# greysun/GraphEmbeddings

Hardware: AMD Instinct MI355X
Metric: scored triples/sec/GPU (d=200) (higher is better)
Workload: dtype f32

## Files before the change

graphembeddings_amd/csrc/ge_train.hip:

```cpp
#include "ge_prep.h"
#include "ge_launch.h"
#include <algorithm>
#include <cmath>
#include <utility>

namespace ge {

__global__ __launch_bounds__(kPrepThreads) void train_prepare_kernel(
    const int32_t* __restrict__ triples, int64_t T, int64_t first_row, int64_t B, int64_t s0,
    const int32_t* __restrict__ id_to_type, int64_t N, const int64_t* __restrict__ type_offsets,
    int32_t n_types, const int32_t* __restrict__ type_ids, uint64_t seed, uint64_t global_step0,
    int32_t padded_size, int32_t mode, int direct, int n_pass, int bits, int negs, int32_t* __restrict__ prep) {
  extern __shared__ __attribute__((aligned(16))) unsigned long long keys[];
  const PrepLayout L = prep_layout(B, negs);
  const int P = (int)L.P, R = P / kPrepThreads;
  unsigned* hist = reinterpret_cast<unsigned*>(keys + P);
  int* wtot = reinterpret_cast<int*>(hist + kPrepWaves * kMaxRadix);
  const int tid = threadIdx.x, lane = tid & (kWave - 1), wave = tid >> 6;
  const int sub = blockIdx.y;
  const int64_t s = s0 + blockIdx.x;
  const int32_t* pos = triples + 3 * step_row(first_row, T, B, s);
  int32_t* rec = prep + (int64_t)blockIdx.x * L.stride;
  int32_t* neg = rec;
  int32_t* slot_item = rec + L.off_slot;
  int32_t* subrec = rec + L.off_sub + sub * L.sub_stride;
  int32_t* items = subrec + L.off_items;
  int32_t* islots = subrec + L.off_islots;
  const int64_t i0 = (int64_t)sub * kSub;
  const int S = (int)((L.units - i0) < kSub ? (L.units - i0) : kSub);
  const uint64_t step = global_step0 + (uint64_t)s;
  const bool batch_heads = (mode == GE_CORRUPT_BATCH_COIN) ? batch_coin_heads(seed, step) : false;
  constexpr unsigned long long kInvalid = ~0ull;

  if (direct)
    for (int i = tid; i < 6 * S; i += kPrepThreads) slot_item[6 * i0 + i] = -1;

  {
    const StepSource src{pos, B, id_to_type, N, type_offsets, n_types, type_ids, seed, step, padded_size, mode, negs};
    for (int il = tid; il < (int)L.S; il += kPrepThreads) {
      unsigned long long k4[4] = {kInvalid, kInvalid, kInvalid, kInvalid};
      if (il < S) unit_keys(src, i0 + il, batch_heads, neg, k4);
      if (negs > 0) {
#pragma unroll
        for (int X = 0; X < 3; ++X) keys[3 * il + X] = k4[X];
      } else {
#pragma unroll
        for (int X = 0; X < 4; ++X) keys[4 * il + X] = k4[X];
      }
    }
  }
  __syncthreads();

  const int radix = 1 << bits;
  const unsigned dmask = (unsigned)radix - 1u;
  const int seg = kWave * R;
  for (int pass = 0; pass < n_pass; ++pass) {
    const int shift = 32 + pass * bits;
    for (int i = tid; i < radix * kPrepWaves; i += kPrepThreads) hist[i] = 0;
    __syncthreads();
    unsigned long long k[16];
    unsigned off[16];
#pragma unroll
    for (int r = 0; r < 16; ++r) {
      if (r < R) {
        k[r] = keys[wave * seg + r * kWave + lane];
        const unsigned dg = (unsigned)(k[r] >> shift) & dmask;
        unsigned long long peers = ~0ull;
        for (int b = 0; b < bits; ++b) {
          const bool bit = (dg >> b) & 1u;
          const unsigned long long bal = __ballot(bit);
          peers &= bit ? bal : ~bal;
        }
        const unsigned rank = (unsigned)__popcll(peers & ((1ull << lane) - 1ull));
        const unsigned cnt = (unsigned)__popcll(peers);
        unsigned* hp = hist + dg * kPrepWaves + wave;
        const unsigned base = *hp;
        __builtin_amdgcn_wave_barrier();
        if (rank == 0) *hp = base + cnt;
        __builtin_amdgcn_wave_barrier();
        off[r] = base + rank;
      }
    }
    __syncthreads();
    {
      const int q = radix * kPrepWaves / kPrepThreads;
      unsigned loc[4];
      int sum = 0;
      for (int u = 0; u < q; ++u) { loc[u] = hist[tid * q + u]; sum += (int)loc[u]; }
      const int incl = wave_incl_add(sum, lane);
      if (lane == kWave - 1) wtot[wave] = incl;
      __syncthreads();
      int run = incl - sum;
      for (int w = 0; w < wave; ++w) run += wtot[w];
      for (int u = 0; u < q; ++u) { hist[tid * q + u] = (unsigned)run; run += (int)loc[u]; }
    }
    __syncthreads();
#pragma unroll
    for (int r = 0; r < 16; ++r) {
      if (r < R) {
        const unsigned dg = (unsigned)(k[r] >> shift) & dmask;
        keys[hist[dg * kPrepWaves + wave] + off[r]] = k[r];
      }
    }
    __syncthreads();
  }

  auto key_at = [&](int i) -> unsigned long long { return (i >= 0 && i < P) ? keys[i] : kInvalid; };
  int rs_loc[16];
  {
    int carry = -1;
#pragma unroll
    for (int r = 0; r < 16; ++r) {
      if (r < R) {
        const int i = wave * seg + r * kWave + lane;
        const unsigned long long kk = keys[i], kp = key_at(i - 1);
        const bool head = kk != kInvalid && (i == 0 || (uint32_t)(kp >> 32) != (uint32_t)(kk >> 32));
        const int m = max(wave_incl_max(head ? i : -1, lane), carry);
        rs_loc[r] = m;
        carry = __shfl(m, kWave - 1, kWave);
      }
    }
    if (lane == 0) wtot[wave] = carry;
  }
  __syncthreads();
  int prev_max = -1;
  for (int w = 0; w < wave; ++w) prev_max = max(prev_max, wtot[w]);
  __syncthreads();
  unsigned start_mask = 0;
  int idx_loc[16];
  {
    int carry = 0;
#pragma unroll
    for (int r = 0; r < 16; ++r) {
      if (r < R) {
        const int i = wave * seg + r * kWave + lane;
        const unsigned long long kk = keys[i], kp = key_at(i - 1), kn = key_at(i + 1);
        const bool valid = kk != kInvalid;
        const uint32_t row = (uint32_t)(kk >> 32);
        const bool head = valid && (i == 0 || (uint32_t)(kp >> 32) != row);
        const bool sole = direct && head && !(kn != kInvalid && (uint32_t)(kn >> 32) == row);
        const int rs = max(rs_loc[r], prev_max);
        rs_loc[r] = rs;
        const bool start = valid && ((i - rs) % kItemCap) == 0 && !sole;
        if (start) start_mask |= 1u << r;
        if (sole) slot_item[(uint32_t)kk] = kSlotDirect;
        const int incl = wave_incl_add(start ? 1 : 0, lane) + carry;
        idx_loc[r] = incl - (start ? 1 : 0);
        carry = __shfl(incl, kWave - 1, kWave);
      }
    }
    if (lane == 0) wtot[wave] = carry;
  }
  __syncthreads();
  int prev_items = 0, total = 0;
  for (int w = 0; w < kPrepWaves; ++w) { if (w < wave) prev_items += wtot[w]; total += wtot[w]; }
  if (tid == 0) subrec[0] = total;
#pragma unroll
  for (int r = 0; r < 16; ++r) {
    if (r < R && ((start_mask >> r) & 1u)) {
      const int i = wave * seg + r * kWave + lane;
      const uint32_t row = (uint32_t)(keys[i] >> 32);
      const int idx = prev_items + idx_loc[r];
      int e = i + 1;
      while (e < P && (e - i) < kItemCap && keys[e] != kInvalid && (uint32_t)(keys[e] >> 32) == row) ++e;
      const bool more = (e < P && keys[e] != kInvalid && (uint32_t)(keys[e] >> 32) == row);
      const bool multi = (i != rs_loc[r]) || more;
      items[2 * idx] = (int32_t)row;
      items[2 * idx + 1] = (e - i) | (multi ? (1 << 30) : 0);
#pragma unroll
      for (int j = 0; j < kItemCap; ++j)
        islots[idx * kItemCap + j] = (i + j < e) ? (int32_t)(uint32_t)keys[i + j] : -1;
    }
  }
}

template <int NJ, bool COND, bool DET = false>
__global__ __launch_bounds__(kBlock) void apply_sorted_kernel(
    float* __restrict__ table, int d, const int32_t* __restrict__ sub0, int64_t sub_stride, int off_items,
    int off_islots, const int32_t* __restrict__ grad_idx, const float* grad_val, int split,
    float* __restrict__ out2) {
  const int lane = threadIdx.x & (kWave - 1);
  const int wave = (int)(((int64_t)blockIdx.x * blockDim.x + threadIdx.x) >> 6);
  const int nwaves = (int)(((int64_t)gridDim.x * blockDim.x) >> 6);
  const int32_t* subrec = sub0 + (int64_t)blockIdx.y * sub_stride;
  const int32_t* items = subrec + off_items;
  const int32_t* islots = subrec + off_islots;
  const int n_items = subrec[0];
  for (int w = wave; w < n_items; w += nwaves) {
    const int row = items[2 * w], cm = items[2 * w + 1];
    int slot_v = (lane < kItemCap) ? islots[w * kItemCap + lane] : -1;
    const int cnt = cm & 0x3FFFFFFF;
    const bool multi = (cm >> 30) & 1;
    const bool away = row >= split;
    float* dst = away ? out2 + (int64_t)(row - split) * d : table + (int64_t)row * d;
    float base[NJ];
#pragma unroll
    for (int j = 0; j < NJ; ++j) {
      const int c = lane + kWave * j;
      base[j] = (!multi && !away && c < d) ? dst[c] : 0.f;
    }
    const bool act_v = slot_v >= 0 && (!grad_idx || grad_idx[slot_v] >= 0);
    if (slot_v < 0) slot_v = 0;
    const unsigned long long live = __ballot(act_v);
    const bool park = DET && multi && !away;
    if (live == 0ull && !(away && !multi) && !park) continue;
    float acc[NJ];
#pragma unroll
    for (int j = 0; j < NJ; ++j) acc[j] = 0.f;
    for (int o = 0; o < cnt; o += 4) {
      int sl[4];
      bool on[4];
#pragma unroll
      for (int q = 0; q < 4; ++q) {
        const int src_lane = (o + q < cnt) ? (o + q) : o;
        sl[q] = __shfl(slot_v, src_lane, kWave);
        on[q] = (o + q < cnt) && ((live >> (o + q)) & 1ull);
      }
      float v[4][NJ];
#pragma unroll
      for (int q = 0; q < 4; ++q) {
        const float* src = grad_val + (int64_t)sl[q] * d;
#pragma unroll
        for (int j = 0; j < NJ; ++j) {
          const int c = lane + kWave * j;
          v[q][j] = (c < d && (!COND || on[q])) ? src[c] : 0.f;
        }
      }
#pragma unroll
      for (int q = 0; q < 4; ++q)
#pragma unroll
        for (int j = 0; j < NJ; ++j) acc[j] += on[q] ? v[q][j] : 0.f;
    }
    float* parked = const_cast<float*>(grad_val) + (int64_t)__shfl(slot_v, 0, kWave) * d;
#pragma unroll
    for (int j = 0; j < NJ; ++j) {
      const int c = lane + kWave * j;
      if (c < d) {
        if (park) parked[c] = acc[j];
        else if (multi) atomic_add_f32(dst + c, acc[j]);
        else dst[c] = base[j] + acc[j];
      }
    }
  }
}

constexpr int kHotBlock = 512;
template <int NJ>
__global__ __launch_bounds__(kHotBlock) void hot_rows_kernel(
    float* __restrict__ table, int d, const int32_t* __restrict__ sub0, int64_t sub_stride, int off_items, int off_islots,
    int n_sub, const float* __restrict__ grad_val) {
  constexpr int kScan = kWave;
  constexpr int kWv = kHotBlock / kWave;
  __shared__ int heads[kScan];
  __shared__ int n_heads;
  __shared__ float part[kWv - 1][NJ * kWave];
  const int t = threadIdx.x, lane = t & (kWave - 1), wv = t >> 6, tile = blockIdx.y;
  auto sub_of = [&](int tl) { return sub0 + (int64_t)tl * sub_stride; };
  const int32_t* subrec = sub_of(tile);
  const int n_items = subrec[0];
  for (int win = blockIdx.x; win * kScan < n_items; win += gridDim.x) {
  if (t == 0) n_heads = 0;
  __syncthreads();
  const int k = win * kScan + t;
  if (t < kScan && k < n_items) {
    const int32_t* items = subrec + off_items;
    const int row = items[2 * k], cm = items[2 * k + 1];
    if ((cm >> 30) & 1) {
      int prev_row = -1;
      if (k > 0) prev_row = items[2 * (k - 1)];
      else if (tile > 0) { const int32_t* ps = sub_of(tile - 1); const int pn = ps[0]; if (pn > 0) prev_row = ps[off_items + 2 * (pn - 1)]; }
      if (prev_row != row) heads[atomicAdd(&n_heads, 1)] = k;
    }
  }
  __syncthreads();
  const int nh = n_heads;
  auto item_at = [&](int k0, int r, int row, int& first_slot) -> bool {
    int idx = k0 + r, tl = tile;
    const int32_t* sr = subrec;
    int ni = n_items;
    while (idx >= ni) {
      idx -= ni; ++tl;
      if (tl >= n_sub) return false;
      sr = sub_of(tl); ni = sr[0];
    }
    first_slot = sr[off_islots + idx * kItemCap];
    return sr[off_items + 2 * idx] == row;
  };
  constexpr int kInFlight = NJ <= 4 ? 16 : 8;
  auto add_rows = [&](int fs, int n, float (&acc)[NJ]) {
    for (int o = 0; o < n; o += kInFlight) {
      float v[kInFlight][NJ];
#pragma unroll
      for (int q = 0; q < kInFlight; ++q)
        if (o + q < n) {
          const float* src = grad_val + (int64_t)__shfl(fs, o + q, kWave) * d;
#pragma unroll
          for (int j = 0; j < NJ; ++j) { const int c = lane + kWave * j; v[q][j] = src[c < d ? c : 0]; }
        }
#pragma unroll
      for (int q = 0; q < kInFlight; ++q)
        if (o + q < n) {
#pragma unroll
          for (int j = 0; j < NJ; ++j) acc[j] += v[q][j];
        }
    }
  };
  for (int h = wv; h < nh; h += kWv) {
    const int k0 = heads[h];
    const int row = (subrec + off_items)[2 * k0];
    int fs = 0;
    const bool mine = item_at(k0, lane, row, fs);
    const int n = __popcll(__ballot(mine));
    if (n == kWave) continue;
    float acc[NJ];
#pragma unroll
    for (int j = 0; j < NJ; ++j) acc[j] = 0.f;
    add_rows(fs, n, acc);
    float* dst = table + (int64_t)row * d;
#pragma unroll
    for (int j = 0; j < NJ; ++j) { const int c = lane + kWave * j; if (c < d) dst[c] = dst[c] + acc[j]; }
    if (lane == 0) heads[h] = -1;
  }
  __syncthreads();
  for (int h = 0; h < nh; ++h) {
    const int k0 = heads[h];
    if (k0 < 0) continue;
    const int row = (subrec + off_items)[2 * k0];
// ... 183 lines not shown
      for (int q = 0; q < RG; ++q)
        if (o + q < cnt && ((live >> (o + q)) & 1ull)) {
          const int sl = __builtin_amdgcn_readlane(slot_v, o + q);
          const float* src = grad_val + (int64_t)sl * d;
#pragma unroll
          for (int j = 0; j < NJ; ++j) load_vec<VW>(src + col[j], v[q][j]);
        }
#pragma unroll
      for (int q = 0; q < RG; ++q)
        if (o + q < cnt && ((live >> (o + q)) & 1ull)) {
#pragma unroll
          for (int j = 0; j < NJ; ++j)
#pragma unroll
            for (int e = 0; e < VW; ++e) acc[j][e] += v[q][j][e];
        }
    }
    if (live == 0ull && !away) continue;
#pragma unroll
    for (int j = 0; j < NJ; ++j) {
      if (!ok[j]) continue;
      float o_[VW];
#pragma unroll
      for (int e = 0; e < VW; ++e) o_[e] = base[j][e] + acc[j][e];
      store_vec<VW>(dst + col[j], o_);
    }
  }
}

int apply_items_launch(float* table, int d, const TileGeom& G, const int32_t* step_rec, const int32_t* gidx,
                       const float* gval, int split, float* out2, hipStream_t st, hipEvent_t ev_start, hipEvent_t ev_stop,
                       int det) {
  const int grid = grid_for(G.P, kBlock / kWave);
  const int nj = (d + kWave - 1) / kWave;
  const dim3 g((unsigned)grid, (unsigned)G.n_sub);
  auto hot = [&]() -> int {
    const dim3 gh((unsigned)((G.P + kWave - 1) / kWave), (unsigned)G.n_sub);
#define LH(NJ) hipLaunchKernelGGL((hot_rows_kernel<NJ>), gh, dim3(kHotBlock), 0, st, table, d, step_rec + G.off_sub, G.sub_stride, G.off_items, G.off_islots, G.n_sub, gval)
    if (nj <= 1) LH(1); else if (nj <= 2) LH(2); else if (nj <= 4) LH(4); else if (nj <= 8) LH(8); else LH(16);
#undef LH
    return launch_status();
  };
  if (det && nj > 16) return GE_ENOTSUP;
#define LA(NJ)                                                                                                             \
  {                                                                                                                        \
    if (G.n_sub > 1) hipExtLaunchKernelGGL((apply_sorted_kernel<NJ, true>), g, dim3(kBlock), 0, st, ev_start, ev_stop, 0, table, d, step_rec + G.off_sub, G.sub_stride, G.off_items, G.off_islots, gidx, gval, split, out2); \
    else if (det) { hipExtLaunchKernelGGL((apply_sorted_kernel<NJ, false, true>), g, dim3(kBlock), 0, st, ev_start, ev_stop, 0, table, d, step_rec + G.off_sub, G.sub_stride, G.off_items, G.off_islots, gidx, gval, split, out2); return hot(); } \
    else hipExtLaunchKernelGGL((apply_sorted_kernel<NJ, false>), g, dim3(kBlock), 0, st, ev_start, ev_stop, 0, table, d, step_rec + G.off_sub, G.sub_stride, G.off_items, G.off_islots, gidx, gval, split, out2); \
  }
  if (gidx != nullptr || G.n_sub > 1) {
    auto al = [](const void* q, int a) { return q == nullptr || reinterpret_cast<uintptr_t>(q) % a == 0; };
    const int vw = (d % 4 == 0 && al(table, 16) && al(gval, 16) && al(out2, 16)) ? 4 : (d % 2 == 0 && al(table, 8) && al(gval, 8) && al(out2, 8)) ? 2 : 1;
    const int njr = (d / vw + kWave - 1) / kWave;
    const dim3 g((unsigned)(G.n_sub > 1 ? grid_for((G.P + 7) / 8, kBlock / kWave) : grid), (unsigned)G.n_sub);
    const bool one_tile = G.n_sub == 1 && out2 == nullptr;
#define LR(VW, NJ)                                                                                                       \
    {                                                                                                                    \
      if (one_tile) {                                                                                                    \
        constexpr int RW = one_tile_rows(VW * NJ);                                                                       \
        if (det) {                                                                                                       \
          hipExtLaunchKernelGGL((apply_rows_kernel<VW, NJ, true, RW>), g, dim3(kBlock), 0, st, ev_start, ev_stop, 0, table, d, \
                                step_rec + G.off_sub, G.sub_stride, G.off_items, G.off_islots, gidx, gval, split, out2); \
          return hot();                                                                                                  \
        }                                                                                                                \
        hipExtLaunchKernelGGL((apply_rows_kernel<VW, NJ, false, RW>), g, dim3(kBlock), 0, st, ev_start, ev_stop, 0, table, d, \
                              step_rec + G.off_sub, G.sub_stride, G.off_items, G.off_islots, gidx, gval, split, out2);   \
        return launch_status();                                                                                          \
      }                                                                                                                  \
      if (det) {                                                                                                         \
        hipExtLaunchKernelGGL((apply_rows_kernel<VW, NJ, true>), g, dim3(kBlock), 0, st, ev_start, ev_stop, 0, table, d, \
                              step_rec + G.off_sub, G.sub_stride, G.off_items, G.off_islots, gidx, gval, split, out2);   \
        return hot();                                                                                                    \
      }                                                                                                                  \
      hipExtLaunchKernelGGL((apply_rows_kernel<VW, NJ>), g, dim3(kBlock), 0, st, ev_start, ev_stop, 0, table, d, \
                            step_rec + G.off_sub, G.sub_stride, G.off_items, G.off_islots, gidx, gval, split, out2);     \
      return launch_status();                                                                                            \
    }
    if (vw == 4) { if (njr <= 1) LR(4, 1) else if (njr <= 2) LR(4, 2) else if (njr <= 4) LR(4, 4) }
    else if (vw == 2) { if (njr <= 1) LR(2, 1) else if (njr <= 2) LR(2, 2) else if (njr <= 4) LR(2, 4) else if (njr <= 8) LR(2, 8) }
    else { if (njr <= 1) LR(1, 1) else if (njr <= 2) LR(1, 2) else if (njr <= 4) LR(1, 4) else if (njr <= 8) LR(1, 8) else if (njr <= 16) LR(1, 16) }
#undef LR
  }
  if (nj <= 1) LA(1) else if (nj <= 2) LA(2) else if (nj <= 4) LA(4) else if (nj <= 8) LA(8) else if (nj <= 16) LA(16)
  else return GE_ENOTSUP;
#undef LA
  return launch_status();
}

static int apply_sorted_launch(float* table, int d, const PrepLayout& L, const int32_t* step_rec, const int32_t* gidx,
                               const float* gval, hipStream_t st, hipEvent_t ev_start, hipEvent_t ev_stop, int det = 0) {
  return apply_items_launch(table, d, geom_of(L), step_rec, gidx, gval, 0x7FFFFFFF, nullptr, st, ev_start, ev_stop, det);
}

static size_t grad_region_bytes(int64_t B, int32_t d) {
  return align_up(sizeof(float) * 6 * (size_t)B * (size_t)d, 256);
}
HingeWs hinge_ws(void* base, int64_t B, int32_t d) {
  const size_t idx = align_up(sizeof(int32_t) * 6 * (size_t)B, 256);
  return HingeWs{ws_at<int32_t>(base, 0), ws_at<float>(base, idx), idx + grad_region_bytes(B, d)};
}

static bool train_fast_ok(int64_t B, int32_t d) { return B >= 1 && B <= (int64_t)1 << 24 && d <= 1024; }

static int64_t prep_chunk_steps(int64_t B, int64_t negs = 0) {
  const int64_t u = negs > 0 ? (1 + negs) * B : B;
  int64_t c = (32 * kSub) / (u < kSub ? kSub : u);
  const int64_t floor_steps = u <= 32768 ? 16 : u <= 4 * 65536 ? 8 : 2;
  return c < floor_steps ? floor_steps : c;
}

static int grad_ring(int64_t B, int32_t d) {
  const size_t reg = grad_region_bytes(B, d);
  size_t r = ((size_t)64 << 20) / reg + 1;
  if (r < 2) r = 2;
  if (r > 16) r = 16;
  if (r < 4 && 4 * reg <= ((size_t)160 << 20)) r = 4;
  return (int)r;
}
static size_t prep_chunk_bytes(int64_t B, int64_t negs = 0) {
  return align_up(sizeof(int32_t) * (size_t)prep_chunk_steps(B, negs) * (size_t)prep_layout(B, negs).stride, 256);
}
static size_t prep_region_bytes(int64_t B, int64_t negs) {
  return 2 * prep_chunk_bytes(B, negs) + prep_big_scratch_bytes(B, negs, prep_chunk_steps(B, negs));
}
struct TrainWs { HingeWs g; int ring; size_t region_floats; int32_t* prep; size_t bytes; };
static TrainWs train_ws(void* base, int64_t B, int32_t d) {
  const HingeWs g = hinge_ws(base, B, d);
  const size_t region = grad_region_bytes(B, d);
  const int ring = grad_ring(B, d);
  const size_t grad = g.bytes + (size_t)(ring - 1) * region;
  return TrainWs{g, ring, region / sizeof(float), ws_at<int32_t>(base, grad), grad + prep_region_bytes(B, 0)};
}
template <class Need, class Step>
static size_t largest_need_up_to(int64_t B, Need need, Step step) {
  size_t best = need(B);
  int64_t b = 1;
  while (b < B) {
    const auto v = step(b);
    if (step(B) == v) break;
    int64_t lo = b, hi = B;
    while (hi - lo > 1) { const int64_t mid = lo + (hi - lo) / 2; if (step(mid) == v) lo = mid; else hi = mid; }
    best = std::max(best, need(lo));
    b = hi;
  }
  return best;
}

size_t train_ws_bytes(int64_t B, int32_t d) {
  if (!train_fast_ok(B, d)) return hinge_ws(nullptr, B, d).bytes;
  return largest_need_up_to(B, [&](int64_t b) { return train_ws(nullptr, b, d).bytes; },
                            [&](int64_t b) { return std::make_pair(prep_chunk_steps(b), (int64_t)grad_ring(b, d)); });
}

static size_t prep_lds_bytes(const PrepLayout& L) {
  return sizeof(unsigned long long) * (size_t)L.P + sizeof(unsigned) * kPrepWaves * kMaxRadix + sizeof(int) * 32;
}

static int prepare_launch(const StepSeq& q, int64_t s0, int64_t n, const TypeSampler& ts, int direct, int32_t* out,
                          void* scratch, hipStream_t st, int negs = 0) {
  const PrepLayout L = prep_layout(q.B, negs);
  if (L.n_sub > 1)
    return prepare_big_launch(q, s0, n, ts, direct, out, scratch, st, negs);
  const SortBits sb = sort_bits_for(ts.N);
  const int n_pass = sb.n_pass, bits = sb.bits;
  const size_t lds = prep_lds_bytes(L);
  hipError_t e = hipFuncSetAttribute(reinterpret_cast<const void*>(train_prepare_kernel),
                                     hipFuncAttributeMaxDynamicSharedMemorySize, 160 * 1024);
  if (e != hipSuccess) return (int)e;
  hipLaunchKernelGGL(train_prepare_kernel, dim3((unsigned)n, (unsigned)L.n_sub), dim3(kPrepThreads), lds, st, q.triples,
                     q.T, q.first_row, q.B, s0, ts.id_to_type, ts.N, ts.type_offsets, ts.n_types, ts.type_ids, ts.seed,
                     q.global_step0, ts.padded_size, ts.mode, direct, n_pass, bits, negs, out);
  return launch_status();
}

#define GE_HIP_TRY(expr) do { hipError_t e_ = (expr); if (e_ != hipSuccess) return (int)e_; } while (0)

struct Pipeline {
  int device = -1;
  hipStream_t side = nullptr;
  hipEvent_t prep_done[2] = {nullptr, nullptr};
  hipEvent_t buf_free[2] = {nullptr, nullptr};
  bool live = false;
  StepIdentity id = {};
  int64_t next_abs = 0, resident[2] = {-1, -1};
};

int pipeline_create(void** out) {
  Pipeline* p = new Pipeline();
  hipError_t e = hipGetDevice(&p->device);
  if (e == hipSuccess) e = hipStreamCreateWithFlags(&p->side, hipStreamNonBlocking);
  for (int i = 0; i < 2 && e == hipSuccess; ++i) {
    e = hipEventCreateWithFlags(&p->prep_done[i], hipEventDisableTiming);
    if (e == hipSuccess) e = hipEventCreateWithFlags(&p->buf_free[i], hipEventDisableTiming);
  }
  if (e != hipSuccess) { delete p; return (int)e; }
  *out = p;
  return 0;
}
int pipeline_reset(void* h) {
  if (!h) return GE_EINVAL;
  static_cast<Pipeline*>(h)->live = false;
  return 0;
}
int pipeline_destroy(void* h) {
  if (!h) return GE_EINVAL;
  Pipeline* p = static_cast<Pipeline*>(h);
  if (p->side) { (void)hipStreamSynchronize(p->side); (void)hipStreamDestroy(p->side); }
  for (int i = 0; i < 2; ++i) {
    if (p->prep_done[i]) (void)hipEventDestroy(p->prep_done[i]);
    if (p->buf_free[i]) (void)hipEventDestroy(p->buf_free[i]);
  }
  delete p;
  return 0;
}

static inline int64_t norm_row(int64_t first_row, int64_t T, int64_t B) {
  int64_t f = first_row % T;
  if (f + B > T) f = 0;
  return f;
}
static inline bool continues(const StepSeq& a, int64_t done, const StepSeq& b) {
  return b.global_step0 == a.global_step0 + (uint64_t)done &&
         norm_row(b.first_row, b.T, b.B) == step_row(a.first_row, b.T, b.B, done);
}

class PrepCursor {
 public:
  PrepCursor(const StepIdentity& id, Pipeline* handle, int32_t* prep_base, hipStream_t st)
      : id_(id), L_(prep_layout(id.seq.B, id.negs)), K_(prep_chunk_steps(id.seq.B, id.negs)),
        buf_ints_((int64_t)(prep_chunk_bytes(id.seq.B, id.negs) / sizeof(int32_t))), base_(prep_base), st_(st),
        pipe_(handle ? handle : &local_), own_side_(handle != nullptr) {
    id_.seq.first_row = norm_row(id.seq.first_row, id.seq.T, id.seq.B);
  }

  int begin() {
    if (own_side_) {
      int dev = -1;
      GE_HIP_TRY(hipGetDevice(&dev));
      if (dev != pipe_->device) return GE_EINVAL;
      Pipeline* p = pipe_;
      const bool cont = p->live && same_source(p->id, id_) && continues(p->id.seq, p->next_abs, id_.seq);
      if (!cont) {
        p->live = true;
        p->id = id_;
        p->next_abs = 0;
        p->resident[0] = p->resident[1] = -1;
      }
      base_abs_ = p->next_abs;
    } else {
      pipe_->id = id_;
      pipe_->side = st_;
    }
    return 0;
  }

  int step(int64_t s, const int32_t** rec) {
    const int64_t abs_s = base_abs_ + s, chunk = abs_s / K_, in_chunk = abs_s % K_;
    if (s == 0 || in_chunk == 0) {
      int rc = ensure(chunk);
      if (rc) return rc;
      if (own_side_) {
        rc = ensure(chunk + 1);
        if (rc) return rc;
        GE_HIP_TRY(hipStreamWaitEvent(st_, pipe_->prep_done[chunk & 1], 0));
      }
    }
    *rec = base_ + (chunk & 1) * buf_ints_ + in_chunk * L_.stride;
    return 0;
  }

  int finish(int64_t n_steps, const int32_t** last_rec) {
    const int64_t la = base_abs_ + n_steps - 1;
    *last_rec = base_ + ((la / K_) & 1) * buf_ints_ + (la % K_) * L_.stride;
    if (own_side_) {
      GE_HIP_TRY(hipStreamWaitEvent(st_, pipe_->prep_done[((la / K_) + 1) & 1], 0));
      pipe_->next_abs = base_abs_ + n_steps;
    }
    return 0;
  }

  const PrepLayout& layout() const { return L_; }

 private:
  int ensure(int64_t c) {
    const int b = (int)(c & 1);
    if (pipe_->resident[b] == c) return 0;
    if (own_side_) {
      GE_HIP_TRY(hipEventRecord(pipe_->buf_free[b], st_));
      GE_HIP_TRY(hipStreamWaitEvent(pipe_->side, pipe_->buf_free[b], 0));
    }
    int rc = prepare_launch(pipe_->id.seq, c * K_, K_, id_.ts, id_.direct, base_ + b * buf_ints_, base_ + 2 * buf_ints_,
                            pipe_->side, id_.negs);
    if (rc) return rc;
    if (own_side_) GE_HIP_TRY(hipEventRecord(pipe_->prep_done[b], pipe_->side));
    pipe_->resident[b] = c;
    return 0;
  }

  StepIdentity id_;
  PrepLayout L_;
  int64_t K_, buf_ints_;
  int32_t* base_;
  hipStream_t st_;
  Pipeline local_;
  Pipeline* pipe_;
  bool own_side_;
  int64_t base_abs_ = 0;
};

int train_steps_run(float* table, int32_t d, const StepSeq& q, int64_t n_steps, const TypeSampler& ts, float margin,
                    const StepHyper& hp, int model, float* loss, int keep_all_losses, int32_t* neg_ws, void* workspace,
                    size_t workspace_bytes, void** ev_pairs, int ev_kernel, void* pipe_handle, hipStream_t st) {
  const int64_t N = ts.N, B = q.B;
  const float max_norm = hp.max_norm;
  if (n_steps <= 0) return 0;
  const int deterministic = (model & GE_STEP_DETERMINISTIC) ? 1 : 0;
  model &= ~GE_STEP_DETERMINISTIC;
  const bool shape_ok = complex_shape_ok(d, table);
  const bool transform = model == GE_MODEL_HOLE && shape_ok;
  const bool spectral = transform || model == GE_MODEL_HOLE_SPECTRAL;
  const bool hole_direct = (model == GE_MODEL_HOLE && !shape_ok) || model == GE_MODEL_HOLE_DIRECT;
  if (hole_direct ? d > hole_max_dim() : !shape_ok) return (!hole_direct && (d & 1)) ? GE_EINVAL : GE_ENOTSUP;
  if (transform) { int rc = hole_spectral_launch(table, N, d, 0, st); if (rc) return rc; }
  struct BackToReal {
// ... 206 lines not shown
```

Measured before the change: 597.9 million.

## Restructure prep kernel: narrow 32-bit sort keys, padded LDS, batched sampling, scatter islots

Templates the prepare kernel on key width and radix bits. When the row and slot bit widths fit, it packs sort keys into 32 bits, which halves LDS traffic in the radix sort. It pads LDS and histogram indexing to cut bank conflicts. Negative sampling is batched across several units per thread so the dependent global loads can overlap. Run detection moves to contiguous per-thread segments, and islots are written through a scatter instead of a per-item while loop. The risks are added complexity and correctness of the new item indexing.

```diff
diff --git a/graphembeddings_amd/csrc/ge_train.hip b/graphembeddings_amd/csrc/ge_train.hip
--- a/graphembeddings_amd/csrc/ge_train.hip
+++ b/graphembeddings_amd/csrc/ge_train.hip
@@ -6,17 +6,112 @@
 
 namespace ge {
 
+#ifdef GE_EXP_PREP_STAMPS
+constexpr int kPrepStampWords = 16;
+__device__ unsigned long long ge_prep_stamps[64 * kPrepStampWords];
+#define PREP_STAMP(n) do { if (threadIdx.x == 0 && blockIdx.x < 64) ge_prep_stamps[blockIdx.x * kPrepStampWords + (n)] = __builtin_amdgcn_s_memtime(); } while (0)
+#define PREP_WALL(n) do { if (threadIdx.x == 0 && blockIdx.x < 64) ge_prep_stamps[blockIdx.x * kPrepStampWords + (n)] = wall_clock64(); } while (0)
+#define PREP_STAMP_SYNC() __syncthreads()
+#else
+#define PREP_STAMP(n) do { } while (0)
+#define PREP_WALL(n) do { } while (0)
+#define PREP_STAMP_SYNC() do { } while (0)
+#endif
+
+constexpr int kPrepUnits = (int)(kSub / kPrepThreads);
+constexpr uint32_t kNoSlot = ~0u;
+__host__ __device__ constexpr int prep_pad(int i) { return i + (i >> 4); }
+static_assert(kPrepWaves == 16, "histogram rows are addressed as 17 dg + wave");
+
+template <int BITS>
+__device__ __forceinline__ unsigned long long digit_peers(unsigned dg) {
+  uint32_t diff_lo = 0, diff_hi = 0;
+#pragma unroll
+  for (int b = 0; b < BITS; ++b) {
+    const uint32_t mine = (uint32_t)__builtin_amdgcn_sbfe((int)dg, b, 1);
+    const unsigned long long bal = __ballot(mine != 0u);
+    diff_lo |= (uint32_t)bal ^ mine;
+    diff_hi |= (uint32_t)(bal >> 32) ^ mine;
+  }
+  return ~(((unsigned long long)diff_hi << 32) | diff_lo);
+}
+
+__device__ __forceinline__ void draw_units(const StepSource& S, const int64_t (&j)[kPrepUnits], const bool (&on)[kPrepUnits],
+                                           bool batch_heads, int32_t (&p)[kPrepUnits][3], int (&col)[kPrepUnits],
+                                           int32_t (&repl)[kPrepUnits], bool (&drawn)[kPrepUnits], int64_t (&pi)[kPrepUnits],
+                                           int64_t (&kk)[kPrepUnits]) {
+  const uint32_t klo = (uint32_t)S.seed, khi = (uint32_t)(S.seed >> 32);
+  uint64_t stepk[kPrepUnits];
+#pragma unroll
+  for (int u = 0; u < kPrepUnits; ++u) {
+    pi[u] = (S.negs > 0 && j[u] >= S.B) ? (j[u] - S.B) % S.B : j[u];
+    kk[u] = (S.negs > 0 && j[u] >= S.B) ? (j[u] - S.B) / S.B : 0;
+    drawn[u] = on[u] && (S.negs == 0 || j[u] >= S.B);
+    stepk[u] = S.negs > 0 ? S.step * (uint64_t)S.negs + (uint64_t)kk[u] : S.step;
+#pragma unroll
+    for (int X = 0; X < 3; ++X) p[u][X] = on[u] ? S.pos[3 * pi[u] + X] : -1;
+  }
+  int32_t ty[kPrepUnits];
+  bool ok[kPrepUnits];
+#pragma unroll
+  for (int u = 0; u < kPrepUnits; ++u) {
+    const uint32_t slo = (uint32_t)stepk[u], shi = (uint32_t)(stepk[u] >> 32);
+    const uint32_t ilo = (uint32_t)pi[u], ihi = (uint32_t)((uint64_t)pi[u] >> 32);
+    bool heads;
+    if (S.mode == GE_CORRUPT_BATCH_COIN) heads = S.negs > 0 ? batch_coin_heads(S.seed, stepk[u]) : batch_heads;
+    else if (S.mode == GE_CORRUPT_ROW_COIN) heads = (philox_w0(slo, shi, ilo, ihi, klo ^ GE_TAG_SIDE, khi) >> 31) == 0;
+    else heads = (S.mode == GE_CORRUPT_HEADS);
+    col[u] = heads ? 0 : 1;
+    const int32_t x = heads ? p[u][0] : p[u][1];
+    ok[u] = drawn[u] && x >= 0 && x < S.N;
+    ty[u] = ok[u] ? S.id_to_type[x] : -1;
+  }
+  int64_t off[kPrepUnits], end[kPrepUnits];
+#pragma unroll
+  for (int u = 0; u < kPrepUnits; ++u) {
+    ok[u] = ok[u] && ty[u] >= 0 && ty[u] < S.n_types;
+    off[u] = ok[u] ? S.type_offsets[ty[u]] : 0;
+    end[u] = ok[u] ? S.type_offsets[ty[u] + 1] : 0;
+  }
+  int64_t pick[kPrepUnits];
+#pragma unroll
+  for (int u = 0; u < kPrepUnits; ++u) {
+    const uint32_t slo = (uint32_t)stepk[u], shi = (uint32_t)(stepk[u] >> 32);
+    const uint32_t ilo = (uint32_t)pi[u], ihi = (uint32_t)((uint64_t)pi[u] >> 32);
+    uint32_t w = philox_w0(slo, shi, ilo, ihi, klo ^ GE_TAG_SLOT, khi);
+    if (S.padded_size > 0) {
+      const uint32_t slot = w % (uint32_t)S.padded_size;
+      w = philox_w0(slo, shi, (uint32_t)ty[u], slot, klo ^ GE_TAG_PICK, khi);
+    }
+    const uint64_t len = (uint64_t)(end[u] - off[u]);
+    ok[u] = ok[u] && len > 0;
+    pick[u] = off[u] + (int64_t)(((uint64_t)w * len) >> 32);
+  }
+#pragma unroll
+  for (int u = 0; u < kPrepUnits; ++u)
+    repl[u] = ok[u] ? S.type_ids[pick[u]] : -1;
+}
+
+template <class KeyT, int BITS>
 __global__ __launch_bounds__(kPrepThreads) void train_prepare_kernel(
     const int32_t* __restrict__ triples, int64_t T, int64_t first_row, int64_t B, int64_t s0,
     const int32_t* __restrict__ id_to_type, int64_t N, const int64_t* __restrict__ type_offsets,
     int32_t n_types, const int32_t* __restrict__ type_ids, uint64_t seed, uint64_t global_step0,
-    int32_t padded_size, int32_t mode, int direct, int n_pass, int bits, int negs, int32_t* __restrict__ prep) {
-  extern __shared__ __attribute__((aligned(16))) unsigned long long keys[];
+    int32_t padded_size, int32_t mode, int direct, int n_pass, int sbits, int negs, int32_t* __restrict__ prep) {
+  extern __shared__ __attribute__((aligned(16))) unsigned char prep_lds[];
+  constexpr int bits = BITS;
+  KeyT* keys = reinterpret_cast<KeyT*>(prep_lds);
+  uint32_t* words = reinterpret_cast<uint32_t*>(prep_lds);
   const PrepLayout L = prep_layout(B, negs);
   const int P = (int)L.P, R = P / kPrepThreads;
-  unsigned* hist = reinterpret_cast<unsigned*>(keys + P);
-  int* wtot = reinterpret_cast<int*>(hist + kPrepWaves * kMaxRadix);
+  const int PW = prep_pad(P);
+  unsigned* hist = reinterpret_cast<unsigned*>(prep_lds + sizeof(unsigned long long) * (size_t)PW);
+  int* wtot = reinterpret_cast<int*>(hist + (kPrepWaves + 1) * kMaxRadix);
   const int tid = threadIdx.x, lane = tid & (kWave - 1), wave = tid >> 6;
+  const int rshift = sizeof(KeyT) == 8 ? 32 : sbits;
+  const uint32_t smask = sizeof(KeyT) == 8 ? ~0u : ((1u << sbits) - 1u);
+  PREP_WALL(0);
+  PREP_STAMP(1);
   const int sub = blockIdx.y;
   const int64_t s = s0 + blockIdx.x;
   const int32_t* pos = triples + 3 * step_row(first_row, T, B, s);
@@ -30,16 +125,58 @@
   const int S = (int)((L.units - i0) < kSub ? (L.units - i0) : kSub);
   const uint64_t step = global_step0 + (uint64_t)s;
   const bool batch_heads = (mode == GE_CORRUPT_BATCH_COIN) ? batch_coin_heads(seed, step) : false;
-  constexpr unsigned long long kInvalid = ~0ull;
-
-  if (direct)
-    for (int i = tid; i < 6 * S; i += kPrepThreads) slot_item[6 * i0 + i] = -1;
+  constexpr KeyT kInvalid = (KeyT)~(KeyT)0;
+
+  if (direct) {
+    int32_t* f = slot_item + 6 * i0;
+    const int n = 6 * S;
+    const int head = min(n, (int)((16u - ((uint32_t)reinterpret_cast<uintptr_t>(f) & 15u)) & 15u) >> 2);
+    const int nv = (n - head) >> 2;
+    int4* f4 = reinterpret_cast<int4*>(f + head);
+    for (int i = tid; i < nv; i += kPrepThreads) f4[i] = make_int4(-1, -1, -1, -1);
+    if (tid < head) f[tid] = -1;
+    if (tid < n - head - 4 * nv) f[head + 4 * nv + tid] = -1;
+  }
 
   {
     const StepSource src{pos, B, id_to_type, N, type_offsets, n_types, type_ids, seed, step, padded_size, mode, negs};
-    for (int il = tid; il < (int)L.S; il += kPrepThreads) {
-      unsigned long long k4[4] = {kInvalid, kInvalid, kInvalid, kInvalid};
-      if (il < S) unit_keys(src, i0 + il, batch_heads, neg, k4);
+    int64_t j[kPrepUnits], pi[kPrepUnits], kk[kPrepUnits];
+    bool on[kPrepUnits], drawn[kPrepUnits];
+    int32_t p[kPrepUnits][3], repl[kPrepUnits];
+    int col[kPrepUnits];
+#pragma unroll
+    for (int u = 0; u < kPrepUnits; ++u) {
+      const int il = tid + u * kPrepThreads;
+      on[u] = il < S;
+      j[u] = i0 + (on[u] ? il : 0);
+    }
+    draw_units(src, j, on, batch_heads, p, col, repl, drawn, pi, kk);
+#pragma unroll
+    for (int u = 0; u < kPrepUnits; ++u) {
+      const int il = tid + u * kPrepThreads;
+      if (il >= (int)L.S) continue;
+      KeyT k4[4] = {kInvalid, kInvalid, kInvalid, kInvalid};
+      if (on[u]) {
+        const int32_t old = col[u] ? p[u][1] : p[u][0];
+        int32_t t3[3] = {p[u][0], p[u][1], p[u][2]};
+        if (drawn[u]) {
+          if (col[u]) t3[1] = repl[u]; else t3[0] = repl[u];
+          int32_t* o = neg + 3 * (negs > 0 ? kk[u] * B + pi[u] : j[u]);
+          o[0] = t3[0]; o[1] = t3[1]; o[2] = t3[2];
+        }
+        bool bad = t3[0] < 0 || t3[1] < 0 || t3[2] < 0 || t3[0] >= N || t3[1] >= N || t3[2] >= N;
+        if (negs > 0) {
+#pragma unroll
+          for (int X = 0; X < 3; ++X)
+            if (!bad) k4[X] = ((KeyT)(uint32_t)t3[X] << rshift) | (KeyT)(uint32_t)(3 * j[u] + X);
+        } else {
+          bad = bad || old < 0 || old >= N;
+#pragma unroll
+          for (int X = 0; X < 3; ++X)
+            if (!bad) k4[X] = ((KeyT)(uint32_t)p[u][X] << rshift) | (KeyT)(uint32_t)(6 * j[u] + X);
+          if (!bad && repl[u] != old) k4[3] = ((KeyT)(uint32_t)repl[u] << rshift) | (KeyT)(uint32_t)(6 * j[u] + 3 + col[u]);
+        }
+      }
       if (negs > 0) {
 #pragma unroll
         for (int X = 0; X < 3; ++X) keys[3 * il + X] = k4[X];
@@ -50,30 +187,27 @@
     }
   }
   __syncthreads();
+  PREP_STAMP(2);
 
   const int radix = 1 << bits;
   const unsigned dmask = (unsigned)radix - 1u;
   const int seg = kWave * R;
   for (int pass = 0; pass < n_pass; ++pass) {
-    const int shift = 32 + pass * bits;
-    for (int i = tid; i < radix * kPrepWaves; i += kPrepThreads) hist[i] = 0;
+    const int shift = rshift + pass * bits;
+    const bool last_pass = pass == n_pass - 1;
+    for (int i = tid; i < radix * (kPrepWaves + 1); i += kPrepThreads) hist[i] = 0;
     __syncthreads();
-    unsigned long long k[16];
+    KeyT k[16];
     unsigned off[16];
 #pragma unroll
     for (int r = 0; r < 16; ++r) {
       if (r < R) {
         k[r] = keys[wave * seg + r * kWave + lane];
         const unsigned dg = (unsigned)(k[r] >> shift) & dmask;
-        unsigned long long peers = ~0ull;
-        for (int b = 0; b < bits; ++b) {
-          const bool bit = (dg >> b) & 1u;
-          const unsigned long long bal = __ballot(bit);
-          peers &= bit ? bal : ~bal;
-        }
+        const unsigned long long peers = digit_peers<BITS>(dg);
         const unsigned rank = (unsigned)__popcll(peers & ((1ull << lane) - 1ull));
         const unsigned cnt = (unsigned)__popcll(peers);
-        unsigned* hp = hist + dg * kPrepWaves + wave;
+        unsigned* hp = hist + ((dg << 4) + dg) + wave;
         const unsigned base = *hp;
         __builtin_amdgcn_wave_barrier();
         if (rank == 0) *hp = base + cnt;
@@ -82,97 +216,129 @@
       }
     }
     __syncthreads();
+    if (pass == 0) PREP_STAMP(7);
     {
       const int q = radix * kPrepWaves / kPrepThreads;
       unsigned loc[4];
       int sum = 0;
-      for (int u = 0; u < q; ++u) { loc[u] = hist[tid * q + u]; sum += (int)loc[u]; }
+      for (int u = 0; u < q; ++u) { loc[u] = hist[prep_pad(tid * q + u)]; sum += (int)loc[u]; }
       const int incl = wave_incl_add(sum, lane);
       if (lane == kWave - 1) wtot[wave] = incl;
       __syncthreads();
       int run = incl - sum;
       for (int w = 0; w < wave; ++w) run += wtot[w];
-      for (int u = 0; u < q; ++u) { hist[tid * q + u] = (unsigned)run; run += (int)loc[u]; }
+      for (int u = 0; u < q; ++u) { hist[prep_pad(tid * q + u)] = (unsigned)run; run += (int)loc[u]; }
     }
     __syncthreads();
+    if (pass == 0) PREP_STAMP(8);
 #pragma unroll
     for (int r = 0; r < 16; ++r) {
       if (r < R) {
         const unsigned dg = (unsigned)(k[r] >> shift) & dmask;
-        keys[hist[dg * kPrepWaves + wave] + off[r]] = k[r];
+        const int dst = (int)(hist[((dg << 4) + dg) + wave] + off[r]);
+        keys[last_pass ? prep_pad(dst) : dst] = k[r];
       }
     }
     __syncthreads();
-  }
-
-  auto key_at = [&](int i) -> unsigned long long { return (i >= 0 && i < P) ? keys[i] : kInvalid; };
-  int rs_loc[16];
+    if (pass == 0) PREP_STAMP(9);
+  }
+
+  PREP_STAMP(3);
+  const int p0 = tid * R;
+  KeyT k[16];
+#pragma unroll
+  for (int r = 0; r < 16; ++r)
+    if (r < R) k[r] = keys[prep_pad(p0 + r)];
+  const KeyT kprev = p0 > 0 ? keys[prep_pad(p0 - 1)] : kInvalid, knext = p0 + R < P ? keys[prep_pad(p0 + R)] : kInvalid;
+  unsigned head_m = 0, sole_m = 0, tail_m = 0;
+  int last_head = -1;
+#pragma unroll
+  for (int r = 0; r < 16; ++r) {
+    if (r < R) {
+      const int i = p0 + r;
+      const KeyT kk = k[r], kp = r == 0 ? kprev : k[r > 0 ? r - 1 : 0];
+      const KeyT kn = (r + 1 < 16 && r + 1 < R) ? k[r + 1 < 16 ? r + 1 : 15] : knext;
+      const bool valid = kk != kInvalid;
+      const bool head = valid && (i == 0 || (kp >> rshift) != (kk >> rshift));
+      const bool tail = valid && !(kn != kInvalid && (kn >> rshift) == (kk >> rshift));
+      if (head) { head_m |= 1u << r; last_head = i; }
+      if (tail) tail_m |= 1u << r;
+      if (direct && head && tail) sole_m |= 1u << r;
+    }
+  }
+  const int incl_head = wave_incl_max(last_head, lane);
+  int run_start0 = __shfl_up(incl_head, 1, kWave);
+  if (lane == 0) run_start0 = -1;
+  if (lane == kWave - 1) wtot[wave] = incl_head;
+  __syncthreads();
+  for (int w = 0; w < wave; ++w) run_start0 = max(run_start0, wtot[w]);
+  int n_start = 0;
   {
-    int carry = -1;
+    int run_start = run_start0;
 #pragma unroll
     for (int r = 0; r < 16; ++r) {
       if (r < R) {
-        const int i = wave * seg + r * kWave + lane;
-        const unsigned long long kk = keys[i], kp = key_at(i - 1);
-        const bool head = kk != kInvalid && (i == 0 || (uint32_t)(kp >> 32) != (uint32_t)(kk >> 32));
-        const int m = max(wave_incl_max(head ? i : -1, lane), carry);
-        rs_loc[r] = m;
-        carry = __shfl(m, kWave - 1, kWave);
-      }
-    }
-    if (lane == 0) wtot[wave] = carry;
-  }
+        const int i = p0 + r;
+        if ((head_m >> r) & 1u) run_start = i;
+        if (k[r] != kInvalid && ((i - run_start) % kItemCap) == 0 && !((sole_m >> r) & 1u)) ++n_start;
+      }
+    }
+  }
+  const int incl_start = wave_incl_add(n_start, lane);
+  if (lane == kWave - 1) wtot[kPrepWaves + wave] = incl_start;
   __syncthreads();
-  int prev_max = -1;
-  for (int w = 0; w < wave; ++w) prev_max = max(prev_max, wtot[w]);
-  __syncthreads();
-  unsigned start_mask = 0;
-  int idx_loc[16];
+  int item = incl_start - n_start - 1, total = 0;
+  for (int w = 0; w < kPrepWaves; ++w) { const int c = wtot[kPrepWaves + w]; if (w < wave) item += c; total += c; }
+  if (tid == 0) subrec[0] = total;
   {
-    int carry = 0;
+    int run_start = run_start0;
 #pragma unroll
     for (int r = 0; r < 16; ++r) {
       if (r < R) {
-        const int i = wave * seg + r * kWave + lane;
-        const unsigned long long kk = keys[i], kp = key_at(i - 1), kn = key_at(i + 1);
-        const bool valid = kk != kInvalid;
-        const uint32_t row = (uint32_t)(kk >> 32);
-        const bool head = valid && (i == 0 || (uint32_t)(kp >> 32) != row);
-        const bool sole = direct && head && !(kn != kInvalid && (uint32_t)(kn >> 32) == row);
-        const int rs = max(rs_loc[r], prev_max);
-        rs_loc[r] = rs;
-        const bool start = valid && ((i - rs) % kItemCap) == 0 && !sole;
-        if (start) start_mask |= 1u << r;
-        if (sole) slot_item[(uint32_t)kk] = kSlotDirect;
-        const int incl = wave_incl_add(start ? 1 : 0, lane) + carry;
-        idx_loc[r] = incl - (start ? 1 : 0);
-        carry = __shfl(incl, kWave - 1, kWave);
-      }
-    }
-    if (lane == 0) wtot[wave] = carry;
+        const int i = p0 + r;
+        const bool valid = k[r] != kInvalid, sole = (sole_m >> r) & 1u, tail = (tail_m >> r) & 1u;
+        if ((head_m >> r) & 1u) run_start = i;
+        const int at = (i - run_start) % kItemCap;
+        const uint32_t slot = (uint32_t)k[r] & smask;
+        const bool queued = valid && !sole;
+        if (queued && at == 0) ++item;
+        if (sole) slot_item[slot] = kSlotDirect;
+        if (queued && (tail || at == kItemCap - 1)) {
+          const bool multi = (i - at != run_start) || !tail;
+          items[2 * item] = (int32_t)(uint32_t)(k[r] >> rshift);
+          items[2 * item + 1] = (at + 1) | (multi ? (1 << 30) : 0);
+        }
+        words[prep_pad(i)] = slot;
+        words[PW + prep_pad(i)] = queued ? (uint32_t)(item * kItemCap + at) : kNoSlot;
+      }
+    }
+  }
+  if ((reinterpret_cast<uintptr_t>(islots) & 15u) == 0) {
+    int4* f4 = reinterpret_cast<int4*>(islots);
+    for (int i = tid; i < total * (kItemCap / 4); i += kPrepThreads) f4[i] = make_int4(-1, -1, -1, -1);
+  } else {
+    for (int i = tid; i < total * kItemCap; i += kPrepThreads) islots[i] = -1;
   }
   __syncthreads();
-  int prev_items = 0, total = 0;
-  for (int w = 0; w < kPrepWaves; ++w) { if (w < wave) prev_items += wtot[w]; total += wtot[w]; }
-  if (tid == 0) subrec[0] = total;
+  PREP_STAMP(4);
 #pragma unroll
   for (int r = 0; r < 16; ++r) {
-    if (r < R && ((start_mask >> r) & 1u)) {
-      const int i = wave * seg + r * kWave + lane;
-      const uint32_t row = (uint32_t)(keys[i] >> 32);
-      const int idx = prev_items + idx_loc[r];
-      int e = i + 1;
-      while (e < P && (e - i) < kItemCap && keys[e] != kInvalid && (uint32_t)(keys[e] >> 32) == row) ++e;
-      const bool more = (e < P && keys[e] != kInvalid && (uint32_t)(keys[e] >> 32) == row);
-      const bool multi = (i != rs_loc[r]) || more;
-      items[2 * idx] = (int32_t)row;
-      items[2 * idx + 1] = (e - i) | (multi ? (1 << 30) : 0);
-#pragma unroll
-      for (int j = 0; j < kItemCap; ++j)
-        islots[idx * kItemCap + j] = (i + j < e) ? (int32_t)(uint32_t)keys[i + j] : -1;
-    }
-  }
-}
+    if (r < R) {
+      const int i = r * kPrepThreads + tid;
+      const uint32_t w = words[PW + prep_pad(i)];
+      if (w != kNoSlot) islots[w] = (int32_t)words[prep_pad(i)];
+    }
+  }
+  PREP_STAMP_SYNC();
+  PREP_STAMP(5);
+  PREP_WALL(6);
+}
+
+#ifdef GE_EXP_PREP_STAMPS
+extern "C" int ge_exp_prep_stamps(unsigned long long* host_out) {
+  return (int)hipMemcpyFromSymbol(host_out, HIP_SYMBOL(ge_prep_stamps), sizeof(unsigned long long) * 64 * kPrepStampWords);
+}
+#endif
 
 template <int NJ, bool COND, bool DET = false>
 __global__ __launch_bounds__(kBlock) void apply_sorted_kernel(
@@ -662,7 +828,7 @@
 }
 
 static size_t prep_lds_bytes(const PrepLayout& L) {
-  return sizeof(unsigned long long) * (size_t)L.P + sizeof(unsigned) * kPrepWaves * kMaxRadix + sizeof(int) * 32;
+  return sizeof(unsigned long long) * (size_t)prep_pad((int)L.P) + sizeof(unsigned) * (kPrepWaves + 1) * kMaxRadix + sizeof(int) * 32;
 }
 
 static int prepare_launch(const StepSeq& q, int64_t s0, int64_t n, const TypeSampler& ts, int direct, int32_t* out,
@@ -673,12 +839,20 @@
   const SortBits sb = sort_bits_for(ts.N);
   const int n_pass = sb.n_pass, bits = sb.bits;
   const size_t lds = prep_lds_bytes(L);
-  hipError_t e = hipFuncSetAttribute(reinterpret_cast<const void*>(train_prepare_kernel),
-                                     hipFuncAttributeMaxDynamicSharedMemorySize, 160 * 1024);
+  int rbits = 1, sbits = 1;
+  while (((int64_t)1 << rbits) <= ts.N) ++rbits;
+  while (((int64_t)1 << sbits) < 6 * L.S) ++sbits;
+  const bool narrow = rbits + sbits <= 32;
+  using u64 = unsigned long long;
+  auto* kernel = bits == 6   ? (narrow ? train_prepare_kernel<uint32_t, 6> : train_prepare_kernel<u64, 6>)
+                 : bits == 7 ? (narrow ? train_prepare_kernel<uint32_t, 7> : train_prepare_kernel<u64, 7>)
+                             : (narrow ? train_prepare_kernel<uint32_t, 8> : train_prepare_kernel<u64, 8>);
+  if (bits < 6 || bits > 8) return GE_EINVAL;
+  hipError_t e = hipFuncSetAttribute(reinterpret_cast<const void*>(kernel), hipFuncAttributeMaxDynamicSharedMemorySize, 160 * 1024);
   if (e != hipSuccess) return (int)e;
-  hipLaunchKernelGGL(train_prepare_kernel, dim3((unsigned)n, (unsigned)L.n_sub), dim3(kPrepThreads), lds, st, q.triples,
+  hipLaunchKernelGGL(kernel, dim3((unsigned)n, (unsigned)L.n_sub), dim3(kPrepThreads), lds, st, q.triples,
                      q.T, q.first_row, q.B, s0, ts.id_to_type, ts.N, ts.type_offsets, ts.n_types, ts.type_ids, ts.seed,
-                     q.global_step0, ts.padded_size, ts.mode, direct, n_pass, bits, negs, out);
+                     q.global_step0, ts.padded_size, ts.mode, direct, n_pass, sbits, negs, out);
   return launch_status();
 }
 
```

Result: no change. 599.6 million, median of 5 (+0.3%).
